# anonymous-author-918/deq-mpc-corl

Measured on AMD Instinct MI355X. Metric: QP solves/sec at (B,T=20,nx=13,nu=4), higher is better.
Workload: dtype f32

## Files before the change

deq-mpc-corl_amd/csrc/alqp_quad.hip:

```cpp
#ifdef ALQP_BWD_DYN_UNIT
#undef ALQP_PHASE_TIMING
#endif
#include <hip/hip_runtime.h>

#include "alqp_quad.hpp"
#include "alqp_dims.hpp"
#include "alqp_launch.hpp"

#if defined(ALQP_QUAD_F32) == defined(ALQP_QUAD_F64)
#error "compile alqp_quad.hip with exactly one of -DALQP_QUAD_F32, -DALQP_QUAD_F64"
#endif

namespace alqp {

#ifndef ALQP_FUSE_LS
#define ALQP_FUSE_LS 1
#endif
#ifdef ALQP_PHASE_TIMING
__device__ unsigned long long g_phase_cycles[10];
#define QSTAMP(b) qd.stamp(b)
#else
#define QSTAMP(b)
#endif
template <typename real, int NX, int NU, bool TRACE, class Dyn = NoDyn>
__global__ __launch_bounds__(64) __attribute__((amdgpu_waves_per_eu(1, 1))) void k_solve_lin_quad(SolveArgs<real> a, TraceArgs<real> tr, real *ws) {
    using C = QCfg<real, NX, NU>;
    constexpr bool NL = Dyn::ID != 0;
#ifndef ALQP_FUSE_LS_F64
#define ALQP_FUSE_LS_F64 1
#endif
    constexpr bool FUSE_LS = ALQP_FUSE_LS && (sizeof(real) == 4 || ALQP_FUSE_LS_F64) && !NL;
    constexpr int N = C::N;
    if (a.skip && *a.skip != 0.0) return;
    const int lane = threadIdx.x, qi = lane >> 2;
    const int b_raw = blockIdx.x * 16 + qi;
    const bool active = b_raw < a.B;
    {
        int stag = a.stagger;
        const int mode = (a.flags >> 20) & 0xf;
        if ((a.flags >> 24) & 0xff) stag = (a.flags >> 24) & 0xff;
        if (stag > 0) {
            const unsigned hw = __builtin_amdgcn_s_getreg(4 | (0 << 6) | (31 << 11));
            int simd = (hw >> 4) & 3;
            if (mode == 1) simd = simd * 16 + ((hw >> 8) & 0xf);
            if (mode == 2) simd &= 1;
            if (mode == 3) simd = blockIdx.x & 1;
            if (mode == 4) simd = (simd & 1) ^ (blockIdx.x & 1);
            if (mode == 5) simd = (hw >> 8) & 3;
            for (int i = 0; i < simd * stag; ++i) __builtin_amdgcn_s_sleep(16);
        }
    }
#ifdef ALQP_ALIAS_ALL
    const int b = (active ? b_raw : a.B - 1) % ALQP_ALIAS_ALL;
#else
    const int b = active ? b_raw : a.B - 1;
#endif
    const int T = a.T, M = C::M(T);

    Quad<real, NX, NU> qd;
    __shared__ real w_lds[QCfg<real, NX, NU>::WLDS_WORDS];
    qd.wl = w_lds + threadIdx.x;
    qd.q = lane & 3;
    qd.T = T;
    qd.active = active;
    qd.gQd = a.Qd + (size_t)b * T * N;
    qd.gq = a.q + (size_t)b * T * N;
    qd.gF = a.F + (size_t)b * (T - 1) * NX * N;
    qd.gc = a.c + (size_t)b * (T - 1) * NX;
    qd.gx0 = a.x0 + (size_t)b * NX;
    qd.gulo = a.ulo + (size_t)b * a.sb_u;
    qd.guhi = a.uhi + (size_t)b * a.sb_u;
    qd.st_u = a.st_u;
    qd.gz = a.z + (size_t)b * T * N;
    qd.glam = a.lam + (size_t)b * M;
    qd.rec = ws + C::rec_base(b, T);
    qd.gFw = const_cast<real *>(qd.gF);
    qd.dyn_h = a.dyn_h;
    qd.rho = a.rho[b];
    qd.info = 0;
    real phi_prev = a.phi[b];
#ifdef ALQP_PHASE_TIMING
    for (int i = 0; i < 10; ++i) qd.tacc[i] = 0;
#endif
    QSTAMP(-1);
    if (!(a.flags & ALQP_WS_PRIMED)) {
        if constexpr (NL) qd.stage_in(false, false);
        else qd.stage_in(a.max_newton == 0 || a.al_iter == 0 || (a.flags & ALQP_EXIT_IN_KERNEL) ||
                         (!C::PHI0_FWD && (a.flags & ALQP_INIT_MERIT)));
    }
    const bool ref_exit = (a.flags & ALQP_EXIT_IN_KERNEL) != 0;
    int gphase = 0;

    int step_id = 0;
    bool pend = false;
    real alpha_pend = 0;
    int bad = 0;
    real rn2 = 0, phi_next = 0;
    for (int it = 0; it < a.al_iter; ++it) {
        bool phi_from_forward = false;
        if (a.flags & ALQP_INIT_MERIT) {
            if (it > 0) {
                phi_prev = phi_next;
            } else if (C::PHI0_FWD && a.max_newton > 0 && !ref_exit) {
                phi_from_forward = true;
            } else {
                if constexpr (NL) qd.template linearize<Dyn>(real(0), false);
                real p1[1];
                qd.template merit_candidates<1>(p1, true);
                phi_prev = p1[0];
            }
        }
        pend = false;
        double nrm_old = 0;
        int n_done = 0;
        if (ref_exit) {
            int bad0 = 0;
            const real r0 = it == 0 ? qd.rplus2(bad0) : rn2;
            nrm_old = sqrt(grid_sum_ordered(wave_sum_leaders(exit_term(r0, qor(qd.info)), active && qd.q == 0), a.exit_scratch, gphase));
        }
        for (int st = 0; st < a.max_newton; ++st, ++step_id) {
            real *tg = nullptr;
            if constexpr (TRACE) tg = (tr.g && active) ? tr.g + ((size_t)step_id * a.B + b) * T * N : nullptr;
            QSTAMP(9);
            if constexpr (NL) {
                qd.template linearize<Dyn>(alpha_pend, pend);
                pend = false;
            }
            qd.forward(tg, alpha_pend, pend, (phi_from_forward && st == 0) ? &phi_prev : nullptr);
            real ph[20];
            qd.template backward<FUSE_LS>(ph);
            QSTAMP(-1);
            if constexpr (TRACE) {
                if (tr.d && active) {
                    real *td = tr.d + ((size_t)step_id * a.B + b) * T * N;
                    for (int t = 0; t < T; ++t)
                        for (int j = qd.q; j < N; j += 4) td[t * N + j] = qd.recp(t)[C::wn(C::oY, j)];
                }
            }
            if constexpr (NL) qd.template merit_nonlin<Dyn>(ph);
            else if constexpr (!FUSE_LS) qd.template merit_candidates<20>(ph, false);
            QSTAMP(6);
            int kbest = 0;
            real best = ph[0];
#pragma unroll
            for (int k = 1; k < 20; ++k) {
                if (k < a.n_ls && !(best != best) && (ph[k] != ph[k] || ph[k] < best)) {
                    best = ph[k];
                    kbest = k;
                }
            }
            const bool acc = best < phi_prev;
            if constexpr (TRACE) {
                if (active && qd.q == 0) {
                    if (tr.phi)
#pragma unroll
                        for (int k = 0; k < 20; ++k)
                            if (k < a.n_ls) tr.phi[((size_t)step_id * a.n_ls + k) * a.B + b] = ph[k];
                    if (tr.phi_prev) tr.phi_prev[(size_t)step_id * a.B + b] = phi_prev;
                    if (tr.k) tr.k[(size_t)step_id * a.B + b] = kbest;
                    if (tr.accept) tr.accept[(size_t)step_id * a.B + b] = acc ? 1 : 0;
                }
            }
            const real alpha = acc ? real(1) / real(1 << kbest) : real(0);
            pend = true;
            alpha_pend = alpha;
            QSTAMP(7);
            phi_prev = best;
            if (ref_exit) {
                int bad1 = 0;
                real ph_unused = 0, r1 = 0;
                qd.template iter_end<Dyn>(alpha_pend, pend, false, (real)a.rho_scale, false, ph_unused, r1, bad1);
                pend = false;
                const double nw = sqrt(grid_sum_ordered(wave_sum_leaders(exit_term(r1, qor(qd.info)), active && qd.q == 0), a.exit_scratch, gphase));
                ++n_done;
                if (nw < a.exit_tol || fabs(nrm_old - nw) / nw < a.exit_tol) break;
                nrm_old = nw;
            }
        }
        if (ref_exit && a.newton_counts && blockIdx.x == 0 && lane == 0) a.newton_counts[it] = grid_barrier_timed_out(a.exit_scratch) ? -1 : n_done;
        bad = 0;
        qd.template iter_end<Dyn>(alpha_pend, pend, (a.flags & ALQP_DUAL_UPDATE) != 0, (real)a.rho_scale, it + 1 == a.al_iter,
                    phi_next, rn2, bad);
        pend = false;
    }
    if (a.al_iter <= 0) {
        rn2 = qd.rplus2(bad);
        qd.stage_out();
    }
#ifdef ALQP_PHASE_TIMING
    QSTAMP(9);
    if (lane == 0)
        for (int i = 0; i < 10; ++i) atomicAdd(&g_phase_cycles[i], qd.tacc[i]);
#endif
    if (active && qd.q == 0) {
        a.rho[b] = qd.rho;
        a.phi[b] = phi_prev;
        if (a.rnorm2) a.rnorm2[b] = rn2;
        if (a.info && qd.info && a.info[b] == 0) a.info[b] = qd.info;
        if (a.status) a.status[b] = bad ? 0 : 1;
    }
}

template <typename real, int NX, int NU, bool DYN = false>
__global__ __launch_bounds__(64) __attribute__((amdgpu_waves_per_eu(1, 1))) void k_backward_quad(BwdArgs<real, DYN> a, real *ws) {
    using C = QCfg<real, NX, NU>;
    constexpr int N = C::N;
    const int lane = threadIdx.x, qi = lane >> 2;
    const int b_raw = blockIdx.x * 16 + qi;
    const bool active = b_raw < a.B;
    const int b = active ? b_raw : a.B - 1;
    const int T = a.T;
    Quad<real, NX, NU> qd;
    __shared__ real w_lds[QCfg<real, NX, NU>::WLDS_WORDS];
    qd.wl = w_lds + threadIdx.x;
    qd.q = lane & 3;
    qd.T = T;
    qd.active = active;
    qd.gF = a.F + (size_t)b * (T - 1) * NX * N;
    qd.gQd = nullptr; qd.gq = nullptr; qd.gc = nullptr; qd.gx0 = nullptr; qd.gulo = nullptr; qd.guhi = nullptr;
    qd.st_u = 0;
    qd.gz = nullptr; qd.glam = nullptr;
    qd.rec = ws + C::rec_base(b, T);
    qd.rho = a.rho[b];
    qd.info = 0;
    qd.solve_forward(a.gbar + (size_t)b * T * N);
    real unused[20];
    qd.template backward<false>(unused);
    if (active) {
        const real *zf = a.z_final + (size_t)b * T * N;
        real *qg = a.q_grad + (size_t)b * T * N;
        real *Qg = a.Qd_grad + (size_t)b * T * N;
        for (int t = 0; t < T; ++t)
            for (int j = qd.q; j < N; j += 4) {
                const real w = qd.recp(t)[C::wn(C::oY, j)];
                qg[t * N + j] = w;
                Qg[t * N + j] = w * zf[t * N + j];
            }
    }
    if constexpr (DYN) {
        constexpr int SW = C::SW;
        const real rho = qd.rho;
        const size_t bd = (size_t)b * (T - 1) * NX;
        const real *zf = a.z_final + (size_t)b * T * N;
        const real *lm = a.lam ? a.lam + (size_t)b * a.sb_lam : nullptr;
        for (int t = 0; t + 1 < T; ++t) {
            real wt[N], wnx[SW];
            qd.ld_rep_n(qd.recp(t) + C::oY, wt);
            qd.ld_ownx_of_n(qd.recp(t + 1) + C::oY, wnx);
            real zt[N];
            if (a.dF) gload<N>(zf + t * N, zt);
#pragma unroll
            for (int s = 0; s < SW; ++s) {
                const int r = 4 * s + qd.q;
                const bool own = (4 * s + 3 < NX || r < NX) && active;
                const int rc = (4 * s + 3 < NX || r < NX) ? r : NX - 1;
                real fr[N];
                gload<N>(qd.gF + ((size_t)t * NX + rc) * N, fr);
                real p = 0;
#pragma unroll
                for (int k = 0; k < N; ++k) p = fma_(fr[k], wt[k], p);
                const real si = wnx[s] - p;
                if (a.dF) {
                    const real v = lm[t * NX + rc];
                    real row[N];
#pragma unroll
                    for (int k = 0; k < N; ++k) row[k] = -v * wt[k] - rho * si * zt[k];
                    if (own) qd.template gstore<N>(a.dF + (bd + (size_t)t * NX + r) * N, row);
                }
                if (a.dc && own) a.dc[bd + (size_t)t * NX + r] = -rho * si;
            }
        }
        if (a.dx0) {
            real w0[SW];
            qd.ld_ownx_of_n(qd.recp(0) + C::oY, w0);
#pragma unroll
            for (int s = 0; s < SW; ++s) {
                const int r = 4 * s + qd.q;
                if ((4 * s + 3 < NX || r < NX) && active) a.dx0[(size_t)b * NX + r] = -rho * w0[s];
            }
        }
    }
}

template <typename real, int NX, int NU>
__global__ __launch_bounds__(64) __attribute__((amdgpu_waves_per_eu(1, 1))) void k_newton_step_quad(StepArgs<real> a, real *ws) {
    using C = QCfg<real, NX, NU>;
    constexpr int N = C::N, SW = C::SW;
    const int lane = threadIdx.x, qi = lane >> 2;
    const int b_raw = blockIdx.x * 16 + qi;
    const bool active = b_raw < a.B;
    const int b = active ? b_raw : a.B - 1;
    const int T = a.T, M = C::M(T) + T * a.nobs;
    Quad<real, NX, NU> qd;
    __shared__ real w_lds[QCfg<real, NX, NU>::WLDS_WORDS];
    qd.wl = w_lds + threadIdx.x;
    qd.q = lane & 3;
    qd.T = T;
    qd.active = active;
    qd.gQd = a.Qd + (size_t)b * T * N;
    qd.gq = a.q + (size_t)b * T * N;
    qd.gF = a.F + (size_t)b * (T - 1) * NX * N;
    qd.gc = nullptr;
    qd.gx0 = a.x0 + (size_t)b * NX;
    qd.gulo = a.ulo + (size_t)b * a.sb_u;
    qd.guhi = a.uhi + (size_t)b * a.sb_u;
    qd.st_u = a.st_u;
    qd.gz = const_cast<real *>(a.z) + (size_t)b * T * N;
    qd.glam = const_cast<real *>(a.lam) + (size_t)b * M;
    qd.rec = ws + C::rec_base(b, T);
    qd.gFw = const_cast<real *>(qd.gF);
    qd.dyn_h = 0;
    qd.rho = a.rho[b];
    qd.info = 0;
    qd.nobs = a.nobs;
    qd.gobs = a.nobs > 0 ? a.obs + (size_t)b * T * a.nobs * 3 : nullptr;
    qd.obs_r2 = a.obs_r2;
    qd.no_init = a.no_init != 0;
    const real *gxn = a.xnext + (size_t)b * (T - 1) * NX;
    real *tg = (a.g_out && active) ? a.g_out + (size_t)b * T * N : nullptr;
    qd.template forward<true>(tg, real(0), false, nullptr, gxn);
    real unused[20];
    qd.template backward<false>(unused, a.d_out + (size_t)b * T * N);
    if (active) {
        if (qd.q == 0 && a.info && qd.info && a.info[b] == 0) a.info[b] = qd.info;
    }
}


template <typename real, int NX, int NU, typename Fn, typename... Args>
int launch_quad_kernel(Fn fn, int B, hipStream_t stream, Args... args) {
    const unsigned grid = (unsigned)((B + 15) / 16);
    return launch_maybe_coop(fn, grid, 0, stream, args...);
}

template <typename real>
int dispatch_solve_quad(int nx, int nu, const SolveArgs<real> &a, const TraceArgs<real> *tr, real *ws,
                        hipStream_t stream) {
    return for_dims(nx, nu, ALQP_E_UNSUPPORTED, [&](auto NX, auto NU) {
        if (tr) return launch_quad_kernel<real, NX, NU>(k_solve_lin_quad<real, NX, NU, true>, a.B, stream, a, *tr, ws);
        return launch_quad_kernel<real, NX, NU>(k_solve_lin_quad<real, NX, NU, false>, a.B, stream, a, TraceArgs<real>{}, ws);
    });
}

template <typename real, bool DYN>
int dispatch_backward_quad(int nx, int nu, const BwdArgs<real, DYN> &a, real *ws, hipStream_t stream) {
    return for_dims(nx, nu, ALQP_E_UNSUPPORTED, [&](auto NX, auto NU) {
        return launch_quad_kernel<real, NX, NU>(k_backward_quad<real, NX, NU, DYN>, a.B, stream, a, ws);
    });
}

template <typename real>
int dispatch_solve_nonlin(int dyn_id, int nx, int nu, const SolveArgs<real> &a, real *ws, hipStream_t stream) {
    if (dyn_id == DynPendulum1l<real>::ID && nx == 2 && nu == 1)
        return launch_quad_kernel<real, 2, 1>(k_solve_lin_quad<real, 2, 1, false, DynPendulum1l<real>>, a.B, stream, a,
                                              TraceArgs<real>{}, ws);
    if (dyn_id == DynCartpole1l<real>::ID && nx == 4 && nu == 1)
        return launch_quad_kernel<real, 4, 1>(k_solve_lin_quad<real, 4, 1, false, DynCartpole1l<real>>, a.B, stream, a,
                                              TraceArgs<real>{}, ws);
    if (dyn_id == DynCartpole1l<real, 2>::ID && nx == 4 && nu == 1)
        return launch_quad_kernel<real, 4, 1>(k_solve_lin_quad<real, 4, 1, false, DynCartpole1l<real, 2>>, a.B, stream, a,
                                              TraceArgs<real>{}, ws);
    if (dyn_id == DynCartpole2l<real>::ID && nx == 6 && nu == 1)
        return launch_quad_kernel<real, 6, 1>(k_solve_lin_quad<real, 6, 1, false, DynCartpole2l<real>>, a.B, stream, a,
                                              TraceArgs<real>{}, ws);
    return ALQP_E_UNSUPPORTED;
}

template <typename real>
int dispatch_step_quad(int nx, int nu, const StepArgs<real> &a, real *ws, hipStream_t stream) {
    return for_dims(nx, nu, ALQP_E_UNSUPPORTED, [&](auto NX, auto NU) {
        return launch_quad_kernel<real, NX, NU>(k_newton_step_quad<real, NX, NU>, a.B, stream, a, ws);
    });
}

#ifdef ALQP_QUAD_F32
using quad_real = float;
#else
using quad_real = double;
#endif
#ifndef ALQP_BWD_DYN_UNIT
template int dispatch_solve_quad<quad_real>(int, int, const SolveArgs<quad_real> &, const TraceArgs<quad_real> *, quad_real *, hipStream_t);
template int dispatch_backward_quad<quad_real, false>(int, int, const BwdArgs<quad_real, false> &, quad_real *, hipStream_t);
template int dispatch_solve_nonlin<quad_real>(int, int, int, const SolveArgs<quad_real> &, quad_real *, hipStream_t);
template int dispatch_step_quad<quad_real>(int, int, const StepArgs<quad_real> &, quad_real *, hipStream_t);
#else
template int dispatch_backward_quad<quad_real, true>(int, int, const BwdArgs<quad_real, true> &, quad_real *, hipStream_t);
#endif

}

#if defined(ALQP_PHASE_TIMING) && defined(ALQP_QUAD_F32)
extern "C" int alqp_debug_phase_cycles(unsigned long long *out10, int reset) {
    if (out10 && hipMemcpyFromSymbol(out10, HIP_SYMBOL(alqp::g_phase_cycles), 10 * sizeof(unsigned long long)) != hipSuccess) return -1;
    if (reset) {
        unsigned long long z[10] = {0};
        if (hipMemcpyToSymbol(HIP_SYMBOL(alqp::g_phase_cycles), z, sizeof(z)) != hipSuccess) return -1;
    }
    return 0;
}
#endif
```

deq-mpc-corl_amd/csrc/alqp_quad.hpp:

```cpp
#pragma once
#include <hip/hip_runtime.h>

#include <type_traits>

#include "alqp_team.hpp"
#include "alqp_dyn.hpp"

namespace alqp {

template <int Q>
__device__ inline float qb(float v) {
    return __builtin_bit_cast(float, __builtin_amdgcn_mov_dpp(__builtin_bit_cast(int, v), Q * 0x55, 0xF, 0xF, true));
}
template <int Q>
__device__ inline double qb(double v) {
    long long b = __builtin_bit_cast(long long, v);
    int lo = __builtin_amdgcn_mov_dpp((int)(b & 0xffffffffll), Q * 0x55, 0xF, 0xF, true);
    int hi = __builtin_amdgcn_mov_dpp((int)(b >> 32), Q * 0x55, 0xF, 0xF, true);
    return __builtin_bit_cast(double, ((long long)hi << 32) | (unsigned int)lo);
}
template <typename real>
__device__ inline real qbv(real v, int src) {
    switch (src & 3) {
        case 0: return qb<0>(v);
        case 1: return qb<1>(v);
        case 2: return qb<2>(v);
        default: return qb<3>(v);
    }
}
template <int CTRL>
__device__ inline float qperm(float v) {
    return __builtin_bit_cast(float, __builtin_amdgcn_mov_dpp(__builtin_bit_cast(int, v), CTRL, 0xF, 0xF, true));
}
template <int CTRL>
__device__ inline double qperm(double v) {
    long long b = __builtin_bit_cast(long long, v);
    int lo = __builtin_amdgcn_mov_dpp((int)(b & 0xffffffffll), CTRL, 0xF, 0xF, true);
    int hi = __builtin_amdgcn_mov_dpp((int)(b >> 32), CTRL, 0xF, 0xF, true);
    return __builtin_bit_cast(double, ((long long)hi << 32) | (unsigned int)lo);
}
template <typename real>
__device__ inline real qsum(real v) {
    v += qperm<0xB1>(v);
    v += qperm<0x4E>(v);
    return v;
}
__device__ inline int qor(int v) {
    v |= __builtin_amdgcn_mov_dpp(v, 0xB1, 0xF, 0xF, true);
    v |= __builtin_amdgcn_mov_dpp(v, 0x4E, 0xF, 0xF, true);
    return v;
}
template <typename real>
__device__ inline real sel4(real a0, real a1, real a2, real a3, int q) {
    real lo = (q & 1) ? a1 : a0, hi = (q & 1) ? a3 : a2;
    return (q & 2) ? hi : lo;
}

struct __attribute__((packed, aligned(4))) f4u { float x, y, z, w; };
struct __attribute__((packed, aligned(8))) d4u { double x, y, z, w; };
__device__ inline void gld4(const float *p, float &a, float &b, float &c, float &d) {
    f4u t = *reinterpret_cast<const f4u *>(p);
    a = t.x; b = t.y; c = t.z; d = t.w;
}
__device__ inline void gld4(const double *p, double &a, double &b, double &c, double &d) {
    d4u t = *reinterpret_cast<const d4u *>(p);
    a = t.x; b = t.y; c = t.z; d = t.w;
}
__device__ inline void gst4(float *p, float a, float b, float c, float d) {
    f4u t; t.x = a; t.y = b; t.z = c; t.w = d;
    *reinterpret_cast<f4u *>(p) = t;
}
__device__ inline void gst4(double *p, double a, double b, double c, double d) {
    d4u t; t.x = a; t.y = b; t.z = c; t.w = d;
    *reinterpret_cast<d4u *>(p) = t;
}
template <int LEN, typename real>
__device__ inline void gload(const real *p, real (&dst)[LEN]) {
#pragma unroll
    for (int c = 0; c + 4 <= LEN; c += 4) gld4(p + c, dst[c], dst[c + 1], dst[c + 2], dst[c + 3]);
#pragma unroll
    for (int c = (LEN / 4) * 4; c < LEN; ++c) dst[c] = p[c];
}

#ifndef ALQP_W_LDS
#define ALQP_W_LDS 1
#endif
#ifndef ALQP_EXP_NOQ
#define ALQP_EXP_NOQ 0
#endif
#ifndef ALQP_EXP_NORS
#define ALQP_EXP_NORS 0
#endif
#ifndef ALQP_EXP_NOL
#define ALQP_EXP_NOL 0
#endif
template <typename real, int SW, int N, bool IN_LDS>
struct WPanel {
    real a[SW][N];
    __device__ __forceinline__ real (&operator[](int s))[N] { return a[s]; }
    __device__ __forceinline__ const real (&operator[](int s) const)[N] { return a[s]; }
};
template <typename real, int N>
struct WRowLds {
    real *p;
    __device__ __forceinline__ real &operator[](int k) const { return p[k * 64]; }
};
template <typename real, int SW, int N>
struct WPanel<real, SW, N, true> {
    real *base;
    __device__ __forceinline__ WRowLds<real, N> operator[](int s) const { return WRowLds<real, N>{base + s * N * 64}; }
};
template <int LEN, typename real>
__device__ __forceinline__ void gload(const real *p, WRowLds<real, LEN> row) {
    real tmp[LEN];
    gload<LEN>(p, tmp);
#pragma unroll
    for (int k = 0; k < LEN; ++k) row[k] = tmp[k];
}

struct NoDyn {
    static constexpr int ID = 0;
};

struct Fld {
    int h, t;
};
template <int H, int T>
struct FldT {
    static constexpr int h = H, t = T;
    __host__ __device__ constexpr operator Fld() const { return {H, T}; }
};
template <typename real>
struct FRef {
    real *p;
    Fld f;
};
template <typename real, int H, int T>
__device__ __forceinline__ FRef<std::remove_const_t<real>> operator+(real *p, FldT<H, T>) {
    return {const_cast<std::remove_const_t<real> *>(p), Fld{H, T}};
}

template <typename real, int NX_, int NU_>
struct QCfg {
    static constexpr int NX = NX_, NU = NU_, N = NX_ + NU_;
    static constexpr int SH = (N + 3) / 4;
    static constexpr int SW = (NX + 3) / 4;
    static constexpr int SY = SH;
    static constexpr int HT = 2 * SH * (SH + 1);
    __host__ __device__ static constexpr int hidx(int s, int j) { return 2 * s * (s + 1) + j; }
    static constexpr int ST = 2 * SW * (SW + 1);
    static constexpr int BLK = 64 / (int)sizeof(real);
#ifndef ALQP_REC_IL_F32
#define ALQP_REC_IL_F32 2
#endif
    static constexpr int IL = sizeof(real) == 4 ? ALQP_REC_IL_F32 : 1;
    static_assert(IL == 1 || BLK == 16, "groups of 16 words are 64-byte blocks");
    __host__ __device__ static constexpr int w(int x) { return (x / 16) * (16 * IL) + x % 16; }
    static constexpr int NLAST = N - 4 * (SH - 1);
    __host__ __device__ static constexpr int lanes_of(int s) { return s == SH - 1 ? NLAST : 4; }
    __host__ __device__ static constexpr int lstride(int s) { return lanes_of(s) == 3 ? 16 : 4 * lanes_of(s); }
    __host__ __device__ static constexpr int lbase(int s) {
        int o = 0;
        for (int i = 0; i < s; ++i) o += (i + 1) * lstride(i);
        return o;
    }
    static constexpr int LW = lbase(SH);
    static constexpr bool PHI0_FWD = sizeof(real) == 4;
#ifndef ALQP_S_AFTER_F32
#define ALQP_S_AFTER_F32 0
#endif
    static constexpr bool S_AFTER = sizeof(real) == 8 || ALQP_S_AFTER_F32;
#ifndef ALQP_W_LDS_F32
#define ALQP_W_LDS_F32 0
#endif
    static constexpr bool W_LDS = ALQP_W_LDS && (sizeof(real) == 8 || ALQP_W_LDS_F32);
    static constexpr int WLDS_WORDS = W_LDS ? SW * N * 64 : 1;
    __host__ __device__ static constexpr int p4(int x) { return (x + 3) & ~3; }
    static constexpr int NF = 9;
    __host__ __device__ static constexpr int fslots(int i) { return (i <= 1 || i == 6 || i == 7) ? SY : (i == 5 ? 4 : SW); }
    static constexpr int oL = 2 * 16 * (SY / 4);
    __host__ __device__ static constexpr int tail_at(int i) {
        int g = (oL + LW + 15) & ~15, o = 0;
        for (int k = 0; k < NF; ++k) {
            const int r = fslots(k) % 4;
            if (r > 0 && o + r > 4) { g += 16; o = 0; }
            if (k == i) return g + o;
            o += r;
        }
        return o > 0 ? g + 16 : g;
    }
    __host__ __device__ static constexpr int head_at(int i) {
        if (i < 2) return i * 16 * (SY / 4);
        int o = tail_at(NF);
        for (int k = 2; k < i; ++k) o += 16 * (fslots(k) / 4);
        return o;
    }
    static constexpr FldT<head_at(0), tail_at(0)> oY{};
    static constexpr FldT<head_at(1), tail_at(1)> oZ{};
    static constexpr FldT<head_at(2), tail_at(2)> oR{};
    static constexpr FldT<head_at(3), tail_at(3)> oS{};
    static constexpr FldT<head_at(4), tail_at(4)> oLE{};
    static_assert(NU <= 4, "the u-slot layout holds one control per lane");
    static constexpr FldT<head_at(5), tail_at(5)> oUS{};
    static constexpr FldT<head_at(6), tail_at(6)> oQ{};
    static constexpr FldT<head_at(7), tail_at(7)> oq{};
    static constexpr FldT<head_at(8), tail_at(8)> oC{};
    static constexpr int RECW = (head_at(NF) + 31) & ~31;
    static_assert(IL == 1 || RECW % 16 == 0, "whole groups per record");
    template <int S>
    __host__ __device__ static constexpr int lp(int m, int q) {
        return m < 4 * (S / 4) ? 16 * (m / 4) + 4 * q + m % 4 : 16 * (S / 4) + q * (S % 4) + m - 4 * (S / 4);
    }
    template <int S>
    __host__ __device__ static constexpr int fw(Fld f, int p) {
        return p < 16 * (S / 4) ? w(f.h + p) : w(f.t + 4 * ((p - 16 * (S / 4)) / (S % 4)) + (p - 16 * (S / 4)) % (S % 4));
    }
    __host__ __device__ static constexpr int pn(int k) { return lp<SY>(k >> 2, k & 3); }
    __host__ __device__ static constexpr int px(int r) { return lp<SW>(r >> 2, r & 3); }
    __host__ __device__ static constexpr int wn(Fld f, int k) { return fw<SY>(f, pn(k)); }
    __host__ __device__ static constexpr int M(int T) { return T * NX + 2 * T * NU; }
    static constexpr int RSTR = RECW * IL;
    __host__ __device__ static constexpr size_t rec_base(int b, int T) { return (size_t)(b / IL) * T * RSTR + (size_t)(b % IL) * 16; }
    __host__ __device__ static constexpr size_t ws_words(int B, int T) { return (size_t)((B + IL - 1) / IL) * T * RSTR; }
    __host__ static bool ws_covers(int B, int T) {
        return rec_base(B - 1, T) + (size_t)(T - 1) * RSTR + w(RECW - 1) + 1 <= ws_words(B, T);
    }
};

template <typename real, int NX, int NU>
struct Quad {
    using C = QCfg<real, NX, NU>;
    static constexpr int N = C::N, SH = C::SH, SW = C::SW, SY = C::SY, HT = C::HT, ST = C::ST, RECW = C::RECW;

    int q, T;
    bool active;
    const real *gQd, *gq, *gF, *gc, *gx0, *gulo, *guhi;
    long st_u;
    real *gz, *glam, *rec;
    real rho;
    int info;
    real *wl;
    using WT = WPanel<real, SW, N, C::W_LDS>;
    __device__ __forceinline__ WT wpanel() const {
        if constexpr (C::W_LDS) return WT{wl};
        else return WT{};
    }
    real *gFw;
    real dyn_h;
    const real *gobs;
    int nobs;
    real obs_r2;
    bool no_init;

    __device__ __forceinline__ real uhi(int t, int j) const { return guhi[t * st_u + j]; }
    __device__ __forceinline__ real ulo(int t, int j) const { return gulo[t * st_u + j]; }
    __device__ __forceinline__ real *recp(int t) const { return rec + (size_t)t * C::RSTR; }
#ifdef ALQP_PHASE_TIMING
    unsigned long long tacc[10], tlast;
    __device__ __forceinline__ void stamp(int bucket) {
        unsigned long long now;
        __builtin_amdgcn_sched_barrier(0);
        asm volatile("s_waitcnt vmcnt(0)\n\ts_memtime %0\n\ts_waitcnt lgkmcnt(0)" : "=s"(now)::"memory");
        __builtin_amdgcn_sched_barrier(0);
        if (bucket >= 0) tacc[bucket] += now - tlast;
        tlast = now;
    }
#define ALQP_STAMP(b) stamp(b)
#else
#define ALQP_STAMP(b)
#endif

    template <int S, int L>
    __device__ __forceinline__ void ld_slots(FRef<real> f, real (&v)[L]) const {
        static_assert(L <= S, "slots of the field");
#pragma unroll
        for (int c = 0; 4 * c < L && c < S / 4; ++c) {
            const real *p = f.p + C::w(f.f.h + 16 * c) + 4 * q;
            if (4 * c + 3 < L) gld4(p, v[4 * c], v[4 * c + 1], v[4 * c + 2], v[4 * c + 3]);
            else
#pragma unroll
                for (int i = 0; 4 * c + i < L; ++i) v[4 * c + i] = p[i];
        }
        constexpr int H = 4 * (S / 4), R = S % 4;
        if constexpr (L > H) {
            const real *p = f.p + C::w(f.f.t) + 4 * q;
#pragma unroll
            for (int m = H; m < L; ++m) v[m] = p[m - H];
        }
    }
    template <int S>
    __device__ __forceinline__ void st_slots(FRef<real> f, const real (&v)[S]) const {
#pragma unroll
        for (int c = 0; c < S / 4; ++c) gst4(f.p + C::w(f.f.h + 16 * c) + 4 * q, v[4 * c], v[4 * c + 1], v[4 * c + 2], v[4 * c + 3]);
        constexpr int H = 4 * (S / 4), R = S % 4;
        if constexpr (R > 0) {
            real *p = f.p + C::w(f.f.t) + 4 * q;
#pragma unroll
            for (int m = H; m < S; ++m) p[m - H] = v[m];
        }
    }
    template <int S>
    __device__ __forceinline__ void ld_field(FRef<real> f, real (&w)[4 * S]) const {
        constexpr int H = 16 * (S / 4), R = S % 4;
#pragma unroll
        for (int c = 0; c < H; c += 4) gld4(f.p + C::w(f.f.h + c), w[c], w[c + 1], w[c + 2], w[c + 3]);
#pragma unroll
        for (int i = H; i < H + 4 * R; ++i) w[i] = f.p[C::template fw<S>(f.f, i)];
    }
    __device__ __forceinline__ void ld_own_n(FRef<real> f, real (&v)[SY]) const { ld_slots<SY, SY>(f, v); }
    __device__ __forceinline__ void ld_own_x(FRef<real> f, real (&v)[SW]) const { ld_slots<SW, SW>(f, v); }
    __device__ __forceinline__ void ld_ownx_of_n(FRef<real> f, real (&v)[SW]) const { ld_slots<SY, SW>(f, v); }
    template <int LEN>
    __device__ __forceinline__ void gstore(real *p, const real (&v)[LEN]) const {
#pragma unroll
        for (int c = 0; c + 4 <= LEN; c += 4) gst4(p + c, v[c], v[c + 1], v[c + 2], v[c + 3]);
#pragma unroll
        for (int c = (LEN / 4) * 4; c < LEN; ++c) p[c] = v[c];
    }
    __device__ __forceinline__ void st_own_n(FRef<real> f, const real (&v)[SY]) const { st_slots<SY>(f, v); }
    __device__ __forceinline__ void st_own_x(FRef<real> f, const real (&v)[SW]) const { st_slots<SW>(f, v); }
    __device__ __forceinline__ void ld_rep_n(FRef<real> f, real (&v)[N]) const {
        real w[4 * SY];
        ld_field<SY>(f, w);
#pragma unroll
        for (int k = 0; k < N; ++k) v[k] = w[C::pn(k)];
    }
    __device__ __forceinline__ void ld_repx_of_n(FRef<real> f, real (&v)[NX]) const {
        real w[4 * SY];
        ld_field<SY>(f, w);
#pragma unroll
        for (int k = 0; k < NX; ++k) v[k] = w[C::pn(k)];
    }
    __device__ __forceinline__ void ld_rep_x(FRef<real> f, real (&v)[NX]) const {
        real w[4 * SW];
        ld_field<SW>(f, w);
#pragma unroll
        for (int r = 0; r < NX; ++r) v[r] = w[C::px(r)];
    }
    __device__ __forceinline__ real *lchunk(real *rp, int s, int c, int ql) const {
        return rp + C::w(C::oL + C::lbase(s) + c * C::lstride(s)) + 4 * ql;
    }
    template <int LEN, int SL>
    __device__ __forceinline__ void own_of(const real (&full)[LEN], real (&v)[SL]) const {
#pragma unroll
        for (int m = 0; m < SL; ++m)
            v[m] = (4 * m < LEN) ? sel4(full[(4 * m < LEN) ? 4 * m : 0], (4 * m + 1 < LEN) ? full[(4 * m + 1 < LEN) ? 4 * m + 1 : 0] : real(0),
                                        (4 * m + 2 < LEN) ? full[(4 * m + 2 < LEN) ? 4 * m + 2 : 0] : real(0),
                                        (4 * m + 3 < LEN) ? full[(4 * m + 3 < LEN) ? 4 * m + 3 : 0] : real(0), q)
                                 : real(0);
    }
    template <int LEN, int SL>
    __device__ __forceinline__ void ld_own_ext(const real *src, real (&v)[SL]) const {
#pragma unroll
        for (int m = 0; m < SL; ++m) {
            const int k = 4 * m + q;
            const real x = src[(4 * m + 3 < LEN || k < LEN) ? k : LEN - 1];
            v[m] = (4 * m + 3 < LEN || k < LEN) ? x : real(0);
        }
    }
    template <int LEN, int SL>
    __device__ __forceinline__ void st_own_ext(real *dst, const real (&v)[SL]) const {
#pragma unroll
        for (int m = 0; m < SL; ++m)
            if (4 * m + 3 < LEN || 4 * m + q < LEN) dst[4 * m + q] = v[m];
    }

    __device__ __forceinline__ int own_ju() const { return (q - NX) & 3; }
    __device__ __forceinline__ void ld_own_us(const real *rp, real &lu, real &ll, real &bu, real &bl) const {
        gld4(rp + C::w(C::oUS.h) + 4 * q, lu, ll, bu, bl);
    }
    __device__ __forceinline__ void st_own_us(real *rp, real lu, real ll, real bu, real bl) const {
        gst4(rp + C::w(C::oUS.h) + 4 * q, lu, ll, bu, bl);
    }
    __device__ __forceinline__ void ld_rep_us(const real *rp, real (&lu)[NU], real (&ll)[NU], real (&bu)[NU], real (&bl)[NU]) const {
        real w[16];
        ld_field<4>(rp + C::oUS, w);
#pragma unroll
        for (int ju = 0; ju < NU; ++ju) {
            const int ql = (NX + ju) & 3;
            lu[ju] = w[4 * ql];
            ll[ju] = w[4 * ql + 1];
            bu[ju] = w[4 * ql + 2];
            bl[ju] = w[4 * ql + 3];
        }
    }

    __device__ __forceinline__ void load_F_rows(int t, WT &W) const {
        const real *Fg = gF + (size_t)t * NX * N;
#pragma unroll
        for (int s = 0; s < SW; ++s) {
            const int r = 4 * s + q;
            const int rc = (4 * s + 3 < NX) ? r : (r < NX ? r : NX - 1);
            gload<N>(Fg + rc * N, W[s]);
            if (4 * s + 3 >= NX) {
// ... 74 lines not shown
#pragma unroll 2
        for (int t = 0; t < T; ++t) {
            const real *rp = recp(t);
            real vn[SY], vx[SW];
            ld_own_n(rp + C::oZ, vn);
            st_own_ext<N>(gz + t * N, vn);
            ld_own_x(rp + C::oLE, vx);
            st_own_ext<NX>(glam + t * NX, vx);
            {
                real lu, ll, bu, bl;
                ld_own_us(rp, lu, ll, bu, bl);
                const int ju = own_ju();
                if (ju < NU) {
                    glam[T * NX + t * 2 * NU + ju] = lu;
                    glam[T * NX + t * 2 * NU + NU + ju] = ll;
                }
            }
        }
    }

    template <class Dyn>
    __device__ __forceinline__ void linearize(real alpha, bool pend) {
        static_assert(Dyn::NX == NX && Dyn::NU == NU, "model / kernel size mismatch");
        for (int t = 0; t < T; ++t) {
            const bool dyn = t < T - 1;
            real *rp = recp(t);
            const real *rn = recp(dyn ? t + 1 : t);
            real zt[N], dt[N], zn[SW], dn[SW];
            ld_rep_n(rp + C::oZ, zt);
            ld_rep_n(rp + C::oY, dt);
            ld_ownx_of_n(rn + C::oZ, zn);
            ld_ownx_of_n(rn + C::oY, dn);
            if (pend) {
#pragma unroll
                for (int k = 0; k < N; ++k) zt[k] = fma_(alpha, dt[k], zt[k]);
#pragma unroll
                for (int s = 0; s < SW; ++s) zn[s] = fma_(alpha, dn[s], zn[s]);
                if (active) {
                    real zo[SY];
                    own_of<N, SY>(zt, zo);
                    st_own_n(rp + C::oZ, zo);
                }
            }
            if (t == 0) {
                real r0[SW];
#pragma unroll
                for (int s = 0; s < SW; ++s) {
                    const int r = 4 * s + q;
                    const real z0r = sel4(zt[4 * s], (4 * s + 1 < NX) ? zt[(4 * s + 1 < NX) ? 4 * s + 1 : 0] : real(0),
                                          (4 * s + 2 < NX) ? zt[(4 * s + 2 < NX) ? 4 * s + 2 : 0] : real(0),
                                          (4 * s + 3 < NX) ? zt[(4 * s + 3 < NX) ? 4 * s + 3 : 0] : real(0), q);
                    r0[s] = (4 * s + 3 < NX || r < NX) ? z0r - gx0[(r < NX) ? r : NX - 1] : real(0);
                }
                if (active) st_own_x(recp(T - 1) + C::oR, r0);
            }
            if (dyn) {
                constexpr int NTL = (N + 3) / 4;
                real xn[NX], Jl[NX][NTL];
                dyn_value_jac_split<Dyn, real>(zt, dyn_h, q, xn, Jl);
                real co[SW], ro[SW];
#pragma unroll
                for (int s = 0; s < SW; ++s) {
                    const int r = 4 * s + q;
                    real Jr[N];
#pragma unroll
                    for (int k = 0; k < N; ++k)
                        Jr[k] = sel4(qbv(Jl[4 * s][k >> 2], k),
                                     (4 * s + 1 < NX) ? qbv(Jl[(4 * s + 1 < NX) ? 4 * s + 1 : 0][k >> 2], k) : real(0),
                                     (4 * s + 2 < NX) ? qbv(Jl[(4 * s + 2 < NX) ? 4 * s + 2 : 0][k >> 2], k) : real(0),
                                     (4 * s + 3 < NX) ? qbv(Jl[(4 * s + 3 < NX) ? 4 * s + 3 : 0][k >> 2], k) : real(0), q);
                    const real xr = sel4(xn[4 * s], (4 * s + 1 < NX) ? xn[(4 * s + 1 < NX) ? 4 * s + 1 : 0] : real(0),
                                         (4 * s + 2 < NX) ? xn[(4 * s + 2 < NX) ? 4 * s + 2 : 0] : real(0),
                                         (4 * s + 3 < NX) ? xn[(4 * s + 3 < NX) ? 4 * s + 3 : 0] : real(0), q);
                    real c = xr;
#pragma unroll
                    for (int k = 0; k < N; ++k) c = fma_(-Jr[k], zt[k], c);
                    const bool okr = 4 * s + 3 < NX || r < NX;
                    if (okr && active) {
                        real *Fr = gFw + ((size_t)t * NX + r) * N;
#pragma unroll
                        for (int k = 0; k < N; ++k) Fr[k] = Jr[k];
                    }
                    co[s] = okr ? c : real(0);
                    ro[s] = okr ? zn[s] - xr : real(0);
                }
                if (active) {
                    st_own_x(rp + C::oC, co);
                    st_own_x(rp + C::oR, ro);
                }
            }
        }
    }
    template <class Dyn>
    __device__ __forceinline__ void merit_nonlin(real (&phi)[20]) {
        real m[5];
#pragma unroll
        for (int i = 0; i < 5; ++i) m[i] = 0;
        real x0v[NX], li[NX];
        gload<NX>(gx0, x0v);
        ld_rep_x(recp(T - 1) + C::oLE, li);
        const real a0 = sel4(real(1), real(0.5), real(0.25), real(0.125), q);
        for (int t = 0; t < T; ++t) {
            const bool dyn = t < T - 1;
            const real *rp = recp(t), *rn = recp(dyn ? t + 1 : t);
            real zt[N], dt[N], Qt[N], qt[N], zn[NX], dn[NX], le[NX], lu[NU], ll[NU], bu[NU], bl[NU];
            ld_rep_n(rp + C::oZ, zt);
            ld_rep_n(rp + C::oY, dt);
            ld_rep_n(rp + C::oQ, Qt);
            ld_rep_n(rp + C::oq, qt);
            ld_repx_of_n(rn + C::oZ, zn);
            ld_repx_of_n(rn + C::oY, dn);
            ld_rep_x(rp + C::oLE, le);
            ld_rep_us(rp, lu, ll, bu, bl);
            real alpha = a0;
#pragma unroll
            for (int i = 0; i < 5; ++i) {
                real zc[N];
                real acc = 0;
#pragma unroll
                for (int j = 0; j < N; ++j) {
                    zc[j] = fma_(alpha, dt[j], zt[j]);
                    acc = fma_(fma_(real(0.5) * Qt[j], zc[j], qt[j]), zc[j], acc);
                }
#pragma unroll
                for (int ju = 0; ju < NU; ++ju) {
                    const real vu = zc[NX + ju] - bu[ju], vl = bl[ju] - zc[NX + ju];
                    const real cu = fmax_(vu, real(0)), cl = fmax_(vl, real(0));
                    acc += fma_(lu[ju], vu, ll[ju] * vl) + real(0.5) * rho * fma_(cu, cu, cl * cl);
                }
                if (dyn) {
                    real xn[NX];
                    dyn_value<Dyn, real>(zc, dyn_h, xn);
#pragma unroll
                    for (int r = 0; r < NX; ++r) {
                        const real rr = fma_(alpha, dn[r], zn[r]) - xn[r];
                        acc = fma_(fma_(real(0.5) * rho, rr, le[r]), rr, acc);
                    }
                }
                if (t == 0) {
#pragma unroll
                    for (int r = 0; r < NX; ++r) {
                        const real rr = zc[r] - x0v[r];
                        acc = fma_(fma_(real(0.5) * rho, rr, li[r]), rr, acc);
                    }
                }
                m[i] += acc;
                alpha *= real(0.0625);
            }
        }
#pragma unroll
        for (int k = 0; k < 20; ++k) phi[k] = qbv(m[k >> 2], k);
    }

    template <bool EXT = false>
    __device__ __forceinline__ void forward(real *g_out, real alpha, bool pending, real *phi0, const real *gxn = nullptr) {
        real mdist = 0;
        real S[ST], Sy[SW];
        real vpo[SW], Syo[SW];
#pragma unroll
        for (int i = 0; i < ST; ++i) S[i] = 0;
#pragma unroll
        for (int s = 0; s < SW; ++s) Sy[s] = 0;
        {
            real z0[SW], xi[SW], li[SW], r0[SW];
            if constexpr (EXT) {
                ld_own_ext<NX>(gz, z0);
                ld_own_ext<NX>(glam + (T - 1) * NX, li);
            } else {
                ld_ownx_of_n(recp(0) + C::oZ, z0);
                ld_own_x(recp(T - 1) + C::oLE, li);
            }
            ld_own_ext<NX>(gx0, xi);
            if (pending) {
                real d0[SW];
                ld_ownx_of_n(recp(0) + C::oY, d0);
#pragma unroll
                for (int s = 0; s < SW; ++s) z0[s] = fma_(alpha, d0[s], z0[s]);
            }
#pragma unroll
            for (int s = 0; s < SW; ++s) {
                bool valid = 4 * s + 3 < NX || 4 * s + q < NX;
                if constexpr (EXT) valid = valid && !no_init;
                const real r = valid ? z0[s] - xi[s] : real(0);
                vpo[s] = valid ? fma_(rho, r, li[s]) : real(0);
                if constexpr (C::PHI0_FWD) mdist += valid ? fma_(fma_(real(0.5) * rho, r, li[s]), r, real(0)) : real(0);
                Syo[s] = 0;
                r0[s] = r;
            }
            if (!EXT && active) st_own_x(recp(T - 1) + C::oR, r0);
        }
        for (int t = 0; t < T; ++t) {
            const bool dyn = t < T - 1;
            WT W = wpanel();
            real Y[N];
            real dio[SY];
            real v[SW];
            real zs[SY];
            real hob[3] = {0, 0, 0};
            real *rp = recp(t);
            {
                real zt[N];
                real Qo[SY], qo[SY];
                real cs[SW], zn[SW], lm[SW];
                real lu, ll, bu, bl;
                const int td = dyn ? t : (T > 1 ? T - 2 : 0);
                const real *rn = recp(td + 1);
                if constexpr (EXT) {
                    ld_own_ext<N>(gz + t * N, zs);
                    ld_own_ext<N>(gQd + t * N, Qo);
                    ld_own_ext<N>(gq + t * N, qo);
                    load_F_rows(td, W);
                    ld_own_ext<NX>(gxn + td * NX, cs);
                    ld_own_ext<NX>(gz + (td + 1) * N, zn);
                    ld_own_ext<NX>(glam + td * NX, lm);
                    const int ju = own_ju(), jc = ju < NU ? ju : 0;
                    const real *lb = glam + T * NX + t * (2 * NU + nobs);
                    const bool has = ju < NU;
                    lu = has ? lb[jc] : real(0);
                    ll = has ? lb[NU + jc] : real(0);
                    bu = has ? guhi[t * st_u + jc] : real(0);
                    bl = has ? gulo[t * st_u + jc] : real(0);
                } else {
                    ld_own_n(rp + C::oZ, zs);
                    if constexpr (ALQP_EXP_NOQ) { for (int m = 0; m < SY; ++m) Qo[m] = real(1); }
                    else ld_own_n(rp + C::oQ, Qo);
                    ld_own_n(rp + C::oq, qo);
                    load_F_rows(td, W);
                    ld_own_x(rp + C::oC, cs);
                    ld_ownx_of_n(rn + C::oZ, zn);
                    ld_own_x(rp + C::oLE, lm);
                    ld_own_us(rp, lu, ll, bu, bl);
                }
                if (pending) {
                    real dt[SY], dn[SW];
                    ld_own_n(rp + C::oY, dt);
                    ld_ownx_of_n(rn + C::oY, dn);
#pragma unroll
                    for (int m = 0; m < SY; ++m) zs[m] = fma_(alpha, dt[m], zs[m]);
#pragma unroll
                    for (int s = 0; s < SW; ++s) zn[s] = fma_(alpha, dn[s], zn[s]);
                }
                ALQP_STAMP(0);
#pragma unroll
                for (int k = 0; k < N; ++k) zt[k] = qbv(zs[k >> 2], k);
                real rro[SW];
                if (!dyn) {
#pragma unroll
                    for (int s = 0; s < SW; ++s)
#pragma unroll
                        for (int k = 0; k < N; ++k) W[s][k] = 0;
                }
#pragma unroll
                for (int s = 0; s < SW; ++s) {
                    const int r = 4 * s + q;
                    real xn = cs[s];
                    if constexpr (!EXT) {
#pragma unroll
                        for (int k = 0; k < N; ++k) xn = fma_(W[s][k], zt[k], xn);
                    }
                    const real rr = zn[s] - xn;
                    const bool ok = dyn && r < NX;
                    v[s] = ok ? fma_(rho, rr, lm[s]) : real(0);
                    rro[s] = ok ? rr : real(0);
                    if constexpr (C::PHI0_FWD) mdist += ok ? fma_(fma_(real(0.5) * rho, rr, lm[s]), rr, real(0)) : real(0);
                }
                if (!ALQP_EXP_NORS && !EXT && dyn && active) st_own_x(rp + C::oR, rro);
                constexpr int MU0 = NX / 4;
                real zu = 0;
#pragma unroll
                for (int m = MU0; m < SY; ++m) zu = (4 * m + q >= NX && 4 * m + q < N) ? zs[m] : zu;
                const real vu = zu - bu, vl = bl - zu;
                const real au = vu >= 0 ? real(1) : real(0), al = vl >= 0 ? real(1) : real(0);
                const real cu = fmax_(vu, real(0)), cl = fmax_(vl, real(0));
                const real gu = fma_(rho, cu, lu) - fma_(rho, cl, ll);
                const real du = rho * (au + al);
                if constexpr (C::PHI0_FWD)
                    mdist += own_ju() < NU ? fma_(lu, vu, ll * vl) + real(0.5) * rho * fma_(cu, cu, cl * cl) : real(0);
                real go[SY];
#pragma unroll
                for (int m = 0; m < SY; ++m) {
                    const int j = 4 * m + q;
                    const bool isx = (4 * m + 3 < NX) ? true : (4 * m >= NX ? false : j < NX);
                    const bool isu = (4 * m + 3 < NX) ? false : (j >= NX && j < N);
                    real g = fma_(Qo[m], zs[m], qo[m]);
                    real d = Qo[m];
                    if constexpr (C::PHI0_FWD) mdist = fma_(fma_(real(0.5) * Qo[m], zs[m], qo[m]), zs[m], mdist);
                    g += isx ? vpo[m < SW ? m : 0] : (isu ? gu : real(0));
                    bool pinned = isx;
                    if constexpr (EXT) {
                        pinned = isx && !(no_init && t == 0);
                        if (no_init && isu) g = 0;
                    }
                    d += pinned ? rho : (isu ? du : real(0));
                    dio[m] = d;
                    go[m] = g;
                }
                if constexpr (EXT && NX >= 3) {
                    if (nobs > 0) {
                        const real *lk = glam + T * NX + t * (2 * NU + nobs) + 2 * NU;
                        real gob = 0;
                        for (int k = 0; k < nobs; ++k) {
                            const real *o = gobs + (size_t)(t * nobs + k) * 3;
                            const real d0 = zt[0] - o[0], d1 = zt[1] - o[1], d2 = zt[2] - o[2];
                            const real ck = obs_r2 - fma_(d0, d0, fma_(d1, d1, d2 * d2));
                            const real dh = q == 0 ? d0 : (q == 1 ? d1 : d2);
                            gob = fma_(fma_(rho, ck > 0 ? ck : real(0), lk[k]), real(-2) * dh, gob);
                            if (ck >= 0) {
                                const real w4 = real(4) * rho * dh;
                                hob[0] = fma_(w4, d0, hob[0]); hob[1] = fma_(w4, d1, hob[1]); hob[2] = fma_(w4, d2, hob[2]);
                            }
                        }
                        go[0] += q < 3 ? gob : real(0);
                    }
                }
#pragma unroll
                for (int m = 0; m < SY; ++m) {
                    const bool isx = (4 * m + 3 < NX) ? true : (4 * m >= NX ? false : 4 * m + q < NX);
                    go[m] = -go[m] - (isx ? Syo[m < SW ? m : 0] : real(0));
                }
                real fv[N];
#pragma unroll
                for (int j = 0; j < N; ++j) {
                    real p = 0;
                    if (dyn) {
#pragma unroll
                        for (int s = 0; s < SW; ++s) p = fma_(W[s][j], v[s], p);
                        p = qsum(p);
                    }
                    fv[j] = p;
                    Y[j] = qbv(go[j >> 2], j) + p;
                }
                if (g_out) {
                    real fo[SY];
                    own_of<N, SY>(fv, fo);
#pragma unroll
                    for (int m = 0; m < SY; ++m) {
                        const bool isx = (4 * m + 3 < NX) ? true : (4 * m >= NX ? false : 4 * m + q < NX);
                        if (4 * m + 3 < N || 4 * m + q < N)
                            g_out[t * N + 4 * m + q] = -(go[m] + fo[m]) - (isx ? Syo[m < SW ? m : 0] : real(0));
                    }
                }
            }
            real H[HT];
#pragma unroll
            for (int i = 0; i < HT; ++i) H[i] = 0;
#pragma unroll
            for (int s = 0; s < SH; ++s)
#pragma unroll
                for (int c = 0; c < 4; ++c)
                    if (4 * s + c < N) H[C::hidx(s, 4 * s + c)] = (q == c) ? dio[s] : real(0);
            if constexpr (EXT && NX >= 3) {
                if (nobs > 0 && q < 3) {
#pragma unroll
                    for (int j = 0; j < 3; ++j) H[C::hidx(0, j)] += hob[j];
                }
            }
            if (t > 0) {
#pragma unroll
                for (int s = 0; s < SW; ++s)
#pragma unroll
                    for (int b = 0; b < 4 * s + 4; ++b)
                        if (b < NX) H[C::hidx(s, b)] -= S[C::hidx(s, b)];
            }
#pragma unroll
            for (int i = 0; i < ST; ++i) S[i] = 0;
#pragma unroll
            for (int s = 0; s < SW; ++s) Sy[s] = 0;
#pragma unroll
            for (int s = 0; s < SW; ++s)
#pragma unroll
                for (int k = 0; k < N; ++k) W[s][k] *= -rho;
            if (dyn) {
                const real irho = real(1) / rho;
#pragma unroll
                for (int r = 0; r < NX; ++r) {
                    real fr[N];
#pragma unroll
                    for (int j = 0; j < N; ++j) fr[j] = qbv(W[r >> 2][j], r);
#pragma unroll
                    for (int s = 0; s < SH; ++s) {
                        real fi = sel4(fr[4 * s], (4 * s + 1 < N) ? fr[(4 * s + 1 < N) ? 4 * s + 1 : 0] : real(0),
                                       (4 * s + 2 < N) ? fr[(4 * s + 2 < N) ? 4 * s + 2 : 0] : real(0),
                                       (4 * s + 3 < N) ? fr[(4 * s + 3 < N) ? 4 * s + 3 : 0] : real(0), q) * irho;
#pragma unroll
                        for (int j = 0; j < 4 * s + 4; ++j)
                            if (j < N) H[C::hidx(s, j)] = fma_(fi, fr[j], H[C::hidx(s, j)]);
                    }
                }
            }
            ALQP_STAMP(1);
            real ipv[C::S_AFTER ? N : 1];
#pragma unroll
            for (int j = 0; j < N; ++j) {
                const real p = qbv(H[C::hidx(j >> 2, j)], j);
                if (!(p > 0) && info == 0) info = t * N + j + 1;
                const real ip = rcp_(fabs_(p));
                if constexpr (C::W_LDS) {
                    constexpr int KB = 8;
                    real wj[SW];
#pragma unroll
                    for (int s = 0; s < SW; ++s) wj[s] = W[s][j];
#pragma unroll
                    for (int k0 = j + 1; k0 < N; k0 += KB) {
                        real wv[KB][SW];
#pragma unroll
                        for (int kk = 0; kk < KB; ++kk)
#pragma unroll
                            for (int s = 0; s < SW; ++s)
                                if (k0 + kk < N) wv[kk][s] = W[s][k0 + kk];
                        __builtin_amdgcn_sched_barrier(0);
#pragma unroll
                        for (int kk = 0; kk < KB; ++kk) {
                            const int k = k0 + kk;
                            if (k < N) {
                                const real lkj = qbv(H[C::hidx(k >> 2, j)], k) * ip;
#pragma unroll
                                for (int s = (k >> 2); s < SH; ++s) H[C::hidx(s, k)] = fma_(-H[C::hidx(s, j)], lkj, H[C::hidx(s, k)]);
#pragma unroll
                                for (int s = 0; s < SW; ++s) W[s][k] = fma_(-wj[s], lkj, wv[kk][s]);
                                Y[k] = fma_(-Y[j], lkj, Y[k]);
                            }
                        }
                    }
                } else {
#pragma unroll
                for (int k = j + 1; k < N; ++k) {
                    const real lkj = qbv(H[C::hidx(k >> 2, j)], k) * ip;
#pragma unroll
                    for (int s = (k >> 2); s < SH; ++s) H[C::hidx(s, k)] = fma_(-H[C::hidx(s, j)], lkj, H[C::hidx(s, k)]);
#pragma unroll
                    for (int s = 0; s < SW; ++s) W[s][k] = fma_(-W[s][j], lkj, W[s][k]);
                    Y[k] = fma_(-Y[j], lkj, Y[k]);
                }
                }
                if constexpr (C::S_AFTER) ipv[j] = ip;
                if (!C::S_AFTER && dyn) {
#pragma unroll
                    for (int b = 0; b < NX; ++b) {
                        const real wbj = qbv(W[b >> 2][j], b) * ip;
#pragma unroll
                        for (int s = (b >> 2); s < SW; ++s) S[C::hidx(s, b)] = fma_(W[s][j], wbj, S[C::hidx(s, b)]);
                    }
                    const real yip = Y[j] * ip;
#pragma unroll
                    for (int s = 0; s < SW; ++s) Sy[s] = fma_(W[s][j], yip, Sy[s]);
                }
                H[C::hidx(j >> 2, j)] = (q == (j & 3)) ? ip : H[C::hidx(j >> 2, j)];
            }
            ALQP_STAMP(2);
            if (active) {
                if (!(ALQP_EXP_NOL && t >= T - ALQP_EXP_NOL))
#pragma unroll
                for (int s = 0; s < SH; ++s)
#pragma unroll
                    for (int c = 0; c <= s; ++c)
                        if (C::lanes_of(s) == 4 || q < C::lanes_of(s))
                            gst4(lchunk(rp, s, c, q), H[C::hidx(s, 4 * c)],
                                 H[C::hidx(s, 4 * c + 1)], H[C::hidx(s, 4 * c + 2)], H[C::hidx(s, 4 * c + 3)]);
                real yo[SY];
                own_of<N, SY>(Y, yo);
                st_own_n(rp + C::oY, yo);
                if (pending) st_own_n(rp + C::oZ, zs);
            }

            if constexpr (C::S_AFTER) {
                if (dyn) {
#pragma unroll
                    for (int j = 0; j < N; ++j) {
#pragma unroll
                        for (int b = 0; b < NX; ++b) {
                            const real wbj = qbv(W[b >> 2][j], b) * ipv[j];
#pragma unroll
                            for (int s = (b >> 2); s < SW; ++s) S[C::hidx(s, b)] = fma_(W[s][j], wbj, S[C::hidx(s, b)]);
                        }
                        const real yip = Y[j] * ipv[j];
#pragma unroll
                        for (int s = 0; s < SW; ++s) Sy[s] = fma_(W[s][j], yip, Sy[s]);
                    }
                }
            }
#pragma unroll
            for (int s = 0; s < SW; ++s) {
                vpo[s] = v[s];
                Syo[s] = Sy[s];
            }
            ALQP_STAMP(3);
        }
        if constexpr (C::PHI0_FWD) { if (phi0) *phi0 = qsum(mdist); }
    }

    __host__ __device__ static constexpr int lane_lo(int m, int j) { return m == (j >> 2) ? (j & 3) + 1 : 0; }
    __device__ __forceinline__ bool in_lanes(int lo, int hi) const {
        return lo == 0 ? q < hi : (hi == 4 ? q >= lo : (q >= lo && q < hi));
    }
    __device__ __forceinline__ void lsolve_own(const real (&H)[HT], real (&u)[SY]) const {
#pragma unroll
        for (int j = 0; j < N; ++j) {
            const int mj = j >> 2;
            const real wj = qbv(u[mj] * H[C::hidx(mj, j)], j);
#pragma unroll
            for (int m = mj; m < SH; ++m) {
                const int lo = lane_lo(m, j);
                if (lo >= C::lanes_of(m)) continue;
                const real v = fma_(-H[C::hidx(m, j)], wj, u[m]);
                u[m] = lo == 0 ? v : (q >= lo ? v : u[m]);
            }
        }
    }
    __device__ __forceinline__ void ltsolve_own(const real (&H)[HT], const real (&y)[SY], real (&d)[SY], real (&rep)[N]) const {
#pragma unroll
        for (int m = 0; m < SY; ++m) d[m] = 0;
#pragma unroll
        for (int i = N - 1; i >= 0; --i) {
            const int mi = i >> 2;
            real p = 0;
            bool any = false;
#pragma unroll
            for (int m = mi; m < SH; ++m) {
                const int lo = lane_lo(m, i), hi = C::lanes_of(m);
                if (lo >= hi) continue;
                const real h = (lo == 0 && hi == 4) ? H[C::hidx(m, i)] : (in_lanes(lo, hi) ? H[C::hidx(m, i)] : real(0));
                p = any ? fma_(h, d[m], p) : h * d[m];
                any = true;
            }
            real r = y[mi];
// ... 425 lines not shown
```

Before: 6.029 million.

## Compute dynamics Gram update F^T F with MFMA through LDS staging

Replaces the per-row DPP broadcast plus FMA accumulation of rho*W^T W into the Hessian with matrix-core MFMA 16x16x4 f32 products. Each quad writes its W panel to a shared LDS image, the wave runs MFMAs over the 16 problems, then the results are transposed back through LDS and added into H, with a scalar border path for columns past 16. It targets the NX=13, NU=4 f32 case and aims to cut the VALU and cross-lane shuffle cost of the Gram update. In exchange it adds LDS traffic, wave syncs and accumulator registers. The unconditional gram_products call also drops the dyn guard, so timesteps without dynamics rely on W having been zeroed.

```diff
diff --git a/deq-mpc-corl_amd/csrc/alqp_quad.hip b/deq-mpc-corl_amd/csrc/alqp_quad.hip
--- a/deq-mpc-corl_amd/csrc/alqp_quad.hip
+++ b/deq-mpc-corl_amd/csrc/alqp_quad.hip
@@ -58,8 +58,9 @@
     const int T = a.T, M = C::M(T);
 
     Quad<real, NX, NU> qd;
-    __shared__ real w_lds[QCfg<real, NX, NU>::WLDS_WORDS];
+    __shared__ __attribute__((aligned(16))) real w_lds[QCfg<real, NX, NU>::LDS_WORDS];
     qd.wl = w_lds + threadIdx.x;
+    qd.gram = w_lds;
     qd.q = lane & 3;
     qd.T = T;
     qd.active = active;
@@ -211,8 +212,9 @@
     const int b = active ? b_raw : a.B - 1;
     const int T = a.T;
     Quad<real, NX, NU> qd;
-    __shared__ real w_lds[QCfg<real, NX, NU>::WLDS_WORDS];
+    __shared__ __attribute__((aligned(16))) real w_lds[QCfg<real, NX, NU>::LDS_WORDS];
     qd.wl = w_lds + threadIdx.x;
+    qd.gram = w_lds;
     qd.q = lane & 3;
     qd.T = T;
     qd.active = active;
@@ -292,8 +294,9 @@
     const int b = active ? b_raw : a.B - 1;
     const int T = a.T, M = C::M(T) + T * a.nobs;
     Quad<real, NX, NU> qd;
-    __shared__ real w_lds[QCfg<real, NX, NU>::WLDS_WORDS];
+    __shared__ __attribute__((aligned(16))) real w_lds[QCfg<real, NX, NU>::LDS_WORDS];
     qd.wl = w_lds + threadIdx.x;
+    qd.gram = w_lds;
     qd.q = lane & 3;
     qd.T = T;
     qd.active = active;
diff --git a/deq-mpc-corl_amd/csrc/alqp_quad.hpp b/deq-mpc-corl_amd/csrc/alqp_quad.hpp
--- a/deq-mpc-corl_amd/csrc/alqp_quad.hpp
+++ b/deq-mpc-corl_amd/csrc/alqp_quad.hpp
@@ -175,6 +175,22 @@
 #endif
     static constexpr bool W_LDS = ALQP_W_LDS && (sizeof(real) == 8 || ALQP_W_LDS_F32);
     static constexpr int WLDS_WORDS = W_LDS ? SW * N * 64 : 1;
+#ifndef ALQP_GRAM_MFMA
+#define ALQP_GRAM_MFMA 1
+#endif
+#ifndef ALQP_GRAM_MFMA_ALL
+#define ALQP_GRAM_MFMA_ALL 0
+#endif
+    __host__ __device__ static constexpr bool gram_dims(int nx, int nu) {
+        return (nx == 13 && nu == 4) ||
+               (ALQP_GRAM_MFMA_ALL && ((nx == 12 && nu == 4) || (nx == 14 && nu == 4) || (nx == 10 && nu == 3)));
+    }
+    static constexpr bool GRAM_MFMA = ALQP_GRAM_MFMA && sizeof(real) == 4 && !W_LDS && gram_dims(NX, NU);
+    static constexpr int GRAM_ISTR = 16 * 16 + 4;
+    static constexpr int GRAM_WORDS = GRAM_MFMA ? 16 * GRAM_ISTR : 1;
+    static constexpr int LDS_WORDS = WLDS_WORDS > GRAM_WORDS ? WLDS_WORDS : GRAM_WORDS;
+    static_assert(!GRAM_MFMA || (N >= 12 && N <= 20 && NX <= 16), "one 16 x 16 image, at most one border slot");
+    static_assert(GRAM_WORDS * sizeof(real) <= 32 * 1024, "four one-wave workgroups per CU with room to spare");
     __host__ __device__ static constexpr int p4(int x) { return (x + 3) & ~3; }
     static constexpr int NF = 9;
     __host__ __device__ static constexpr int fslots(int i) { return (i <= 1 || i == 6 || i == 7) ? SY : (i == 5 ? 4 : SW); }
@@ -240,6 +256,7 @@
     real rho;
     int info;
     real *wl;
+    real *gram;
     using WT = WPanel<real, SW, N, C::W_LDS>;
     __device__ __forceinline__ WT wpanel() const {
         if constexpr (C::W_LDS) return WT{wl};
@@ -620,6 +637,70 @@
         for (int k = 0; k < 20; ++k) phi[k] = qbv(m[k >> 2], k);
     }
 
+    using f32x4 = __attribute__((ext_vector_type(4))) float;
+    __device__ __forceinline__ void gram_products(const WT &W, f32x4 (&acc)[16]) const {
+        const int lane = threadIdx.x;
+        real *own = gram + (lane >> 2) * C::GRAM_ISTR + 16 * q;
+        wave_sync();
+#pragma unroll
+        for (int s = 0; s < SW; ++s)
+#pragma unroll
+            for (int c = 0; c < 4; ++c) {
+                f32x4 v;
+#pragma unroll
+                for (int e = 0; e < 4; ++e) v[e] = (4 * c + e < N) ? W[s][(4 * c + e < N) ? 4 * c + e : 0] : real(0);
+                *reinterpret_cast<f32x4 *>(own + 64 * s + 4 * c) = v;
+            }
+        wave_sync();
+        const real *op = gram + lane;
+#pragma unroll
+        for (int i = 0; i < 16; ++i) {
+            acc[i] = f32x4{0, 0, 0, 0};
+#pragma unroll
+            for (int kk = 0; kk < SW; ++kk) {
+                const real a = op[i * C::GRAM_ISTR + 64 * kk];
+                acc[i] = __builtin_amdgcn_mfma_f32_16x16x4f32(a, a, acc[i], 0, 0, 0);
+            }
+        }
+        wave_sync();
+    }
+    __device__ __forceinline__ void gram_add(const f32x4 (&acc)[16], real (&H)[HT]) const {
+        const int lane = threadIdx.x;
+        real *tr = gram + 16 * (lane & 15) + 4 * (lane >> 4);
+        wave_sync();
+#pragma unroll
+        for (int i = 0; i < 16; ++i) *reinterpret_cast<f32x4 *>(tr + i * C::GRAM_ISTR) = acc[i];
+        wave_sync();
+        const real *own = gram + (lane >> 2) * C::GRAM_ISTR + 16 * q;
+#pragma unroll
+        for (int m = 0; m < SH && m < 4; ++m)
+#pragma unroll
+            for (int c = 0; c <= m; ++c) {
+                const f32x4 g = *reinterpret_cast<const f32x4 *>(own + 64 * m + 4 * c);
+#pragma unroll
+                for (int e = 0; e < 4; ++e)
+                    if (4 * c + e < N) H[C::hidx(m, 4 * c + e)] = fma_(rho, g[e], H[C::hidx(m, 4 * c + e)]);
+            }
+        wave_sync();
+    }
+    __device__ __forceinline__ void gram_border(const WT &W, real (&H)[HT]) const {
+        if constexpr (SH == 5) {
+#pragma unroll
+            for (int j = 0; j < N; ++j) {
+                real g = 0;
+#pragma unroll
+                for (int c = 0; c < N - 16; ++c) {
+                    real p = W[0][16 + c] * W[0][j];
+#pragma unroll
+                    for (int s = 1; s < SW; ++s) p = fma_(W[s][16 + c], W[s][j], p);
+                    p = qsum(p);
+                    g = (q == c) ? p : g;
+                }
+                H[C::hidx(4, j)] = fma_(rho, g, H[C::hidx(4, j)]);
+            }
+        }
+    }
+
     template <bool EXT = false>
     __device__ __forceinline__ void forward(real *g_out, real alpha, bool pending, real *phi0, const real *gxn = nullptr) {
         real mdist = 0;
@@ -665,6 +746,7 @@
             real v[SW];
             real zs[SY];
             real hob[3] = {0, 0, 0};
+            f32x4 G[C::GRAM_MFMA ? 16 : 1];
             real *rp = recp(t);
             {
                 real zt[N];
@@ -718,6 +800,7 @@
 #pragma unroll
                         for (int k = 0; k < N; ++k) W[s][k] = 0;
                 }
+                if constexpr (C::GRAM_MFMA) gram_products(W, G);
 #pragma unroll
                 for (int s = 0; s < SW; ++s) {
                     const int r = 4 * s + q;
@@ -834,11 +917,15 @@
             for (int i = 0; i < ST; ++i) S[i] = 0;
 #pragma unroll
             for (int s = 0; s < SW; ++s) Sy[s] = 0;
+            if constexpr (C::GRAM_MFMA) {
+                gram_add(G, H);
+                gram_border(W, H);
+            }
 #pragma unroll
             for (int s = 0; s < SW; ++s)
 #pragma unroll
                 for (int k = 0; k < N; ++k) W[s][k] *= -rho;
-            if (dyn) {
+            if (!C::GRAM_MFMA && dyn) {
                 const real irho = real(1) / rho;
 #pragma unroll
                 for (int r = 0; r < NX; ++r) {
```

Result: no change. 6.116 million (median of 6 runs) (+1.4%).
